# drprojects/DeepViewAgg

Measured on AMD Instinct MI355X. Metric: points/sec fused fwd+bwd (1M pts, 32 views), higher is better.
Workload: dtype bf16

## Files before the change

deepviewagg_amd/_lib.py:

```python
import ctypes
import os

_HERE = os.path.dirname(os.path.abspath(__file__))
LIB_PATH = os.environ.get("DVA_LIB_PATH") or os.path.join(_HERE, "csrc", "libdva_hip.so")

DVA_F32, DVA_BF16, DVA_F16 = 0, 1, 2
DVA_GRID_F32, DVA_GRID_F64, DVA_GRID_I32, DVA_GRID_I64 = 0, 1, 2, 3
DVA_SUM, DVA_MEAN, DVA_MAX, DVA_MIN = 0, 1, 2, 3
REDUCE_CODE = {"sum": DVA_SUM, "add": DVA_SUM, "mean": DVA_MEAN, "max": DVA_MAX, "min": DVA_MIN}
CAMERA_CODE = {
    "s3dis_equirectangular": 0,
    "scannet": 1,
    "kitti360_perspective": 2,
    "kitti360_fisheye": 3,
}

_ERRORS = {
    -1: "DVA_ERR_INVALID (bad argument)",
    -2: "DVA_ERR_UNSUPPORTED",
    -3: "DVA_ERR_LAUNCH (HIP runtime error)",
    -4: "DVA_ERR_OVERFLOW (composite key does not fit int64)",
}


# ... 83 lines not shown
    "dva_rowbn_apply": (ctypes.c_int, [_vp, _vp, _vp, _i64, _i32, _f32, _i32, _vp]),
    "dva_rowbn_bwd_stats": (ctypes.c_int, [_vp, _vp, _vp, _vp, _i64, _i32, _f32, _i32, _vp]),
    "dva_rowbn_bwd_apply": (ctypes.c_int, [_vp, _vp, _vp, _vp, _vp, _vp, _i64, _i32, _f32, _i32, _vp]),
    "dva_emod_rows_grid": (ctypes.c_int, [_i64, _i32, _i32]),
    "dva_emod_rows_fwd": (ctypes.c_int, [_vp] * 6 + [_i64, _i32, _i32, _f32, _i32, _vp]),
    "dva_emod_rows_bwd": (ctypes.c_int, [_vp] * 11 + [_i64, _i32, _i32, _f32, _f32, _i32, _vp]),
    "dva_emod_rows_dw_reduce": (ctypes.c_int, [_vp, _i32, _i32, _vp, _vp, _i32, _i32, _vp, _vp]),
    "dva_bn_finalize": (ctypes.c_int, [_vp, ctypes.c_double, _vp, _vp, _vp, _vp, _vp, _f32, _f32, _i32, _i32, _vp,
                                       _vp]),
    "dva_scale_f64": (ctypes.c_int, [_vp, ctypes.c_double, _vp, _i32, _vp]),
    "dva_chain_prep": (ctypes.c_int, [_vp, _vp, _vp, _i32, _vp, _vp, _i32, _vp, _vp]),
    "dva_chain_tile_count": (ctypes.c_int, [_vp, _vp, _i32, _vp, _vp]),
    "dva_chain_tile_build": (ctypes.c_int, [_vp, _vp, _i32, _vp, _vp, _vp]),
    "dva_chain_moments": (ctypes.c_int, [_vp, _i64, _vp, _i32, _vp, _vp, _vp]),
    "dva_chain_stats2": (ctypes.c_int, [_vp, _vp, _vp, _vp, _vp, _vp, _vp, _vp, _vp, _vp, _i64, _vp]),
    "dva_chain_pooled": (ctypes.c_int, [_vp, _vp, _vp, _vp, _i64, _vp]),
    "dva_chain_stats": (ctypes.c_int, [_i32, _vp, _vp, _vp, _vp, _vp, _vp, _vp, _vp, _vp, _vp, _i64, _i64, _vp]),
    "dva_chain_attn_fwd": (ctypes.c_int, [_vp] * 18 + [_i64, _i64, _i64, _i32, _i32, _i32, _f32, _vp]),
    "dva_chain_attn_bwd": (ctypes.c_int, [_vp] * 14 + [_i64, _i64, _i64, _i32, _i32, _i32, _f32, _vp]),
    "dva_chain_attn_fwd_dt": (ctypes.c_int, [_vp] * 18 + [_i64, _i64, _i64, _i32, _i32, _i32, _f32, _i32, _vp]),
    "dva_chain_attn_bwd_dt": (ctypes.c_int, [_vp] * 14 + [_i64, _i64, _i64, _i32, _i32, _i32, _f32, _i32, _vp]),
    "dva_chain_attn_bwd_f32": (ctypes.c_int, [_vp] * 14 + [_i64, _i64, _i64, _i32, _i32, _i32, _f32, _vp]),
    "dva_gather_segment_max_fwd": (ctypes.c_int, [_vp] * 5 + [_i64, _i64, _i64, _i32, _i32, _vp]),
    "dva_gather_segment_max_bwd": (ctypes.c_int, [_vp] * 8 + [_i64, _i64, _i64, _i32, _i32, _vp]),
    "dva_chain_keys_compat": (ctypes.c_int, [_vp] * 14 + [_i32, _f32, _i64, _i64, _vp]),
    "dva_chain_attn_fwd_keys": (ctypes.c_int, [_vp] * 12 + [_f32] + [_vp] * 8 + [_i64, _i64, _i64, _i32, _i32, _i32, _f32, _vp]),
    "dva_qkv_dquery": (ctypes.c_int, [_vp, _i32, _vp, _vp, _vp, _i64, _i64, _i32, _f32, _vp]),
    "dva_chain_score_stats_keys": (ctypes.c_int, [_vp] * 15 + [_i32, _f32, _i64, _i64, _vp]),
    "dva_chain_bwd_layer6_keys": (ctypes.c_int, [_vp] * 16 + [_i32, _f32, _i64, _i64, _vp]),
    "dva_qkv_compat": (ctypes.c_int, [_vp] * 4 + [_i64, _i32, _f32, _vp]),
    "dva_qkv_compat_bwd": (ctypes.c_int, [_vp] * 7 + [_i64, _i64, _i32, _f32, _vp]),
    "dva_plan_split_table_bytes": (ctypes.c_int64, [_i64, _i64]),
    "dva_plan_split_build": (ctypes.c_int, [_vp, _i64, _i64, _vp, _vp, _vp, _i64, _vp, _i64, _vp]),
    "dva_plan_split_sort_records": (ctypes.c_int, [_vp, _vp, _i64, _i64, _vp, _vp, _i64, _vp, _vp, _vp]),
    "dva_plan_split_sort_records32": (ctypes.c_int, [_vp, _vp, _i64, _i64, _vp, _i64, _vp, _vp]),
    "dva_plan_split_rows_grad": (ctypes.c_int, [_vp, _vp, _i64, _i64, _vp, _i64, _vp, _i32, _i32, _i32, _i32, _vp]),
    "dva_chain_score_stats": (ctypes.c_int, [_vp] * 14 + [_i32, _i64, _i64, _vp]),
    "dva_chain_bwd_layer": (ctypes.c_int, [_i32] + [_vp] * 22 + [_i32, _i64, _i64, _vp]),
    "dva_gather_bilinear_taps_anchor": (ctypes.c_int, [_vp, _vp, _i64, _i32, _i32, _i32, _vp, _vp, _vp, _vp]),
    "dva_bilinear_taps_cat": (ctypes.c_int, [_i32, _vp, _vp, _vp, _vp, _vp, _vp, _vp, _i64, _vp, _vp, _vp, _vp]),
    "dva_anchor_rows_sum": (ctypes.c_int, [_vp, _vp, _vp, _vp, _vp, _i64, _i64, _i32, _i32, _vp]),
    "dva_anchor_combine": (ctypes.c_int, [_vp, _vp, _i32, _i32, _i32, _i32, _vp]),
    "dva_anchor_fixup": (ctypes.c_int, [_vp, _vp, _vp, _vp, _vp, _i64, _i32, _i32, _i32, _i32, _i32, _vp]),
    "dva_anchor_rows_sum_bn": (ctypes.c_int, [_vp] * 10 + [_i64, _i64, _i32, _vp]),
    "dva_anchor_fixup_bn": (ctypes.c_int, [_vp] * 8 + [_i64, _i32, _i32, _i32, _i32, _vp]),
    "dva_emod_prep": (ctypes.c_int, [_vp, _i32, _vp, _vp]),
    "dva_emod_stats": (ctypes.c_int, [_i32] + [_vp] * 9 + [_i64, _i64, _i32, _vp]),
    "dva_emod_attn_fwd": (ctypes.c_int, [_vp] * 23 + [_i64, _i64, _i64, _i32, _i32, _i32, _f32, _vp]),
    "dva_emod_attn_bwd": (ctypes.c_int, [_vp] * 20 + [_i64, _i64, _i64, _i32, _i32, _i32, _f32, _vp]),
    "dva_emod_stats1_plan": (ctypes.c_int, [_vp] * 6 + [_i64, _i64, _i32, _vp]),
    "dva_emod_bwd": (ctypes.c_int, [_i32] + [_vp] * 16 + [_i64, _i64, _i64, _i32, _i32, _vp]),
    "dva_chain_route_stats": (ctypes.c_int, [_vp, _vp, _vp, _vp, _vp, _vp, _i64, _vp]),
    "dva_copy_ceiling": (ctypes.c_int, [_vp, _vp, _i64, _vp]),
    "dva_zero_unseen_rows": (ctypes.c_int, [_vp, _vp, _i64, _i64, _vp]),
    "dva_chain_bn_consts": (ctypes.c_int, [_vp, ctypes.c_double, _vp, _vp, _vp, _vp, _vp, ctypes.c_float, ctypes.c_float,
                                           _i32, _vp, _i32, _i32, _vp, _vp, _vp]),
    "dva_concat_cast_fwd": (ctypes.c_int, [_vp, _vp, _vp, _i64, _i32, _i32, _i32, _vp]),
    "dva_concat_cast_bwd": (ctypes.c_int, [_vp, _vp, _vp, _i64, _i32, _i32, _i32, _vp]),
    "dva_mapping_row_index": (ctypes.c_int, [_vp, _vp, _vp, _i32, ctypes.c_double, _i64, _i64, _i32, _i32, _i32, _vp, _vp]),
    "dva_view_gather_rows_grad_rec16_to": (ctypes.c_int, [_vp, _vp, _vp, _vp, _vp, _i32, _i64, _i64, _i32, _i32, _i32, _vp]),
    "dva_chain_tile_chunks": (ctypes.c_int, [_vp, _i64, _i64, _i32, _vp, _vp]),
    "dva_chain_tile_offsets": (ctypes.c_int, [_vp, _i32, _vp, _vp, _vp]),
    "dva_bn_bwd_consts": (ctypes.c_int, [_vp, _vp, ctypes.c_double, _i32, _vp, _vp, _vp, _i32, _vp]),
    "dva_chain3_prep": (ctypes.c_int, [_vp, _vp, _vp, _i32, _vp, _vp, _i32, _vp, _vp]),
    "dva_chain3_stats2": (ctypes.c_int, [_vp] * 11 + [_i64, _vp]),
    "dva_chain3_stats": (ctypes.c_int, [_i32] + [_vp] * 9 + [_i64, _i64, _vp]),
# ... 185 lines not shown
```

deepviewagg_amd/csrc/deepset.hip:

```cpp
#include "dva_common.h"

namespace dva {

constexpr int D = 32;
constexpr int TILE = 32;
constexpr float SLOPE = 0.2f;

struct BNc {
  float mean, invstd, gamma, beta;
};
__device__ __forceinline__ BNc load_bn(const float* __restrict__ bn, int c) {
  BNc b;
  b.mean = bn[c]; b.invstd = bn[D + c]; b.gamma = bn[2 * D + c]; b.beta = bn[3 * D + c];
  return b;
}
__device__ __forceinline__ float bn_hat(float a, const BNc& b) { return (a - b.mean) * b.invstd; }
__device__ __forceinline__ float bn_z(float a, const BNc& b) { return bn_hat(a, b) * b.gamma + b.beta; }
__device__ __forceinline__ float leaky(float z) { return z > 0.f ? z : SLOPE * z; }
__device__ __forceinline__ float dleaky(float z) { return z > 0.f ? 1.f : SLOPE; }

__device__ __forceinline__ void wave_sync() {
  asm volatile("s_waitcnt lgkmcnt(0)" ::: "memory");
  __builtin_amdgcn_wave_barrier();
}
// ... 543 lines not shown
      const int e = i * 64 + lane;
      const int64_t g = row0 * 8 + e;
      s_x[wv][e] = g < V * 8 ? x_map[g] : 0.f;
    }
    wave_sync();
#pragma unroll 4
    for (int i = 0; i < 16; ++i) {
      const int row = 2 * i + h;
      const int64_t r = row0 + row;
      if (r < V) {
        const float a1 = dot_row<8>(&s_x[wv][row * 8], wa);
        const float da = gsc * (Elt<AT>::ld(dz1, r * D + n) - s1m - bn_hat(a1, b) * s2m);
        const float4 x0 = *reinterpret_cast<const float4*>(&s_x[wv][row * 8]);
        const float4 x1 = *reinterpret_cast<const float4*>(&s_x[wv][row * 8 + 4]);
        acc[0] = fmaf(da, x0.x, acc[0]); acc[1] = fmaf(da, x0.y, acc[1]);
        acc[2] = fmaf(da, x0.z, acc[2]); acc[3] = fmaf(da, x0.w, acc[3]);
        acc[4] = fmaf(da, x1.x, acc[4]); acc[5] = fmaf(da, x1.y, acc[5]);
        acc[6] = fmaf(da, x1.z, acc[6]); acc[7] = fmaf(da, x1.w, acc[7]);
      }
    }
    wave_sync();
  }
  for (int i = threadIdx.x; i < D * 8; i += blockDim.x) s_red[i] = 0.f;
  __syncthreads();
#pragma unroll
  for (int k = 0; k < 8; ++k) {
    const float v = acc[k] + __shfl_xor(acc[k], 32);
    if (lane < 32) atomicAdd(&s_red[n * 8 + k], v);
  }
  __syncthreads();
  for (int i = threadIdx.x; i < D * 8; i += blockDim.x) atomicAdd(&dWa[i], s_red[i]);
}

__global__ __launch_bounds__(256) void csr_expand_kernel(const int64_t* __restrict__ ptr, int64_t N,
                                                          int32_t* __restrict__ vp) {
  const int lane = threadIdx.x & 63;
  const int64_t wave = ((int64_t)blockIdx.x * blockDim.x + threadIdx.x) >> 6;
  const int64_t n_waves = ((int64_t)gridDim.x * blockDim.x) >> 6;
  for (int64_t p0 = wave * 64; p0 < N; p0 += n_waves * 64) {
    const int64_t pl = p0 + lane < N ? p0 + lane : N - 1;
    const int64_t b = ptr[pl], e = ptr[pl + 1];
    const int n_here = (int)(N - p0 < 64 ? N - p0 : 64);
    const int64_t first = __shfl(b, 0), last = __shfl(e, n_here - 1);
    if (last - first <= 8 * n_here) {
      if (lane < n_here)
        for (int64_t r = b; r < e; ++r) vp[r] = (int32_t)(p0 + lane);
    } else {
      for (int i = 0; i < n_here; ++i) {
        const int64_t bi = __shfl(b, i), ei = __shfl(e, i);
        for (int64_t r = bi + lane; r < ei; r += 64) vp[r] = (int32_t)(p0 + i);
      }
    }
  }
}

static inline int grid_rows(int64_t V) {
  return capped_grid((V + TILE - 1) / TILE, 4, 256 * 8);
}

int dsm_launch_fwd_first(const float*, const float*, const float*, const float*, void*, double*, int64_t,
                         int, int, hipStream_t);
int dsm_launch_fwd_layer(const void*, const float*, const float*, const float*, const int32_t*, void*,
                         double*, int64_t, int, hipStream_t);
int dsm_launch_fwd_score(const void*, const float*, const float*, const float*, float*, int64_t, int,
                         const float*, const float*, int, hipStream_t);
int dsm_launch_bwd_layer(const void*, const void*, const float*, const float*, const float*, const void*,
                         const float*, const float*, void*, float*, double*, float*, const int32_t*, float*,
                         const float*, int64_t, int, int, int, hipStream_t);
int dsm_launch_bwd_max(const void*, const void*, const float*, const int32_t*, const float*, const int32_t*,
                       void*, double*, int64_t, int, hipStream_t);
int dsm_launch_bwd_score(const float*, const void*, const float*, const float*, void*, float*, float*,
                         double*, int64_t, int, const float*, const float*, int, hipStream_t);

static inline int act_bf(int32_t act_dtype) {
  return act_dtype == DVA_F32 ? 0 : act_dtype == DVA_BF16 ? 1 : -1;
}

}

using namespace dva;

extern "C" {

int dva_csr_expand(const int64_t* ptr, int64_t n_groups, int32_t* group_of_row, void* stream) {
  if (n_groups < 0 || !ptr) return DVA_ERR_INVALID;
  if (n_groups == 0) return DVA_OK;
  if (!group_of_row) return DVA_ERR_INVALID;
  int64_t b = (n_groups + 255) / 256;
  if (b > 8192) b = 8192;
  hipLaunchKernelGGL(csr_expand_kernel, dim3((int)b), dim3(256), 0, (hipStream_t)stream, ptr, n_groups,
                     group_of_row);
  DVA_CHECK_LAUNCH();
  return DVA_OK;
}

int dva_deepset_fwd_first(const float* x_map, const float* Wa, const float* bn1, const float* Wb,
                          void* a2_, double* stats, int64_t V, int32_t F, int32_t stats_only,
                          int32_t algo, int32_t act_dtype, void* stream) {
  const int bf = act_bf(act_dtype);
  if (act_dtype == DVA_F16) return DVA_ERR_UNSUPPORTED;
  if (V < 0 || !stats || bf < 0) return DVA_ERR_INVALID;
  if (bf && algo == 1) return DVA_ERR_UNSUPPORTED;
  float* a2 = (float*)a2_;
  if (F != 8) return DVA_ERR_UNSUPPORTED;
  if (V == 0) return DVA_OK;
  if (!x_map || !Wa) return DVA_ERR_INVALID;
  if (!stats_only && (!bn1 || !Wb || !a2)) return DVA_ERR_INVALID;
  hipStream_t s = (hipStream_t)stream;
  if (algo != 1) {
    dsm_launch_fwd_first(x_map, Wa, bn1, Wb, a2_, stats, V, stats_only, bf, s);
    DVA_CHECK_LAUNCH();
    return DVA_OK;
  }
  if (stats_only) {
    hipLaunchKernelGGL((dsf_fwd_first_kernel<true>), dim3(grid_rows(V)), dim3(256), 0, s, x_map, Wa,
                       (const float*)nullptr, (const float*)nullptr, (float*)nullptr, stats, V);
  } else {
    if (!bn1 || !Wb || !a2) return DVA_ERR_INVALID;
    hipLaunchKernelGGL((dsf_fwd_first_kernel<false>), dim3(grid_rows(V)), dim3(256), 0, s, x_map, Wa,
                       bn1, Wb, a2, stats, V);
  }
  DVA_CHECK_LAUNCH();
  return DVA_OK;
}
// ... 202 lines not shown
```

deepviewagg_amd/csrc/dva_common.h:

```cpp
#pragma once
#include <hip/hip_runtime.h>
#include <stdint.h>

#include "../../include/dva.h"

#define DVA_WAVE 64

#define DVA_CHECK_LAUNCH()                           \
  do {                                               \
    hipError_t e__ = hipGetLastError();              \
    if (e__ != hipSuccess) return DVA_ERR_LAUNCH;    \
  } while (0)

namespace dva {

typedef uint16_t bf16_t;

__device__ __forceinline__ float bf2f(bf16_t h) { return __uint_as_float(((uint32_t)h) << 16); }

typedef __bf16 dva_bf16x2 __attribute__((ext_vector_type(2)));
typedef float dva_f32x2 __attribute__((ext_vector_type(2)));
__device__ __forceinline__ uint32_t pack_bf16x2(float lo, float hi) {
  const dva_f32x2 v = {lo, hi};
  const dva_bf16x2 b = __builtin_convertvector(v, dva_bf16x2);
// ... 50 lines not shown
};
template <>
struct Elt<bf16_t> {
  static __device__ __forceinline__ float ld(const bf16_t* p, int64_t i) { return bf2f(p[i]); }
  static __device__ __forceinline__ void st(bf16_t* p, int64_t i, float v) { p[i] = f2bf(v); }
};
template <>
struct Elt<f16_t> {
  static __device__ __forceinline__ float ld(const f16_t* p, int64_t i) { return (float)p[i]; }
  static __device__ __forceinline__ void st(f16_t* p, int64_t i, float v) { p[i] = (f16_t)v; }
};

__host__ __device__ __forceinline__ int group_of_channel(int c, int C, int G) {
  if (G <= 1) return 0;
  if (G >= C) return c;
  const int base = C / G, rem = C % G;
  const int split = rem * (base + 1);
  return c < split ? c / (base + 1) : rem + (c - split) / base;
}
__host__ __device__ __forceinline__ int group_begin(int g, int C, int G) {
  if (g >= G) return C;
  if (G <= 1) return 0;
  if (G >= C) return g;
  const int base = C / G, rem = C % G;
  return g < rem ? g * (base + 1) : rem * (base + 1) + (g - rem) * base;
}

struct __attribute__((aligned(8))) PackedIdx {
  int32_t img;
  int16_t x;
  int16_t y;
};

static inline int blocks_for(int64_t n, int threads) { return (int)((n + threads - 1) / threads); }

static inline int capped_grid(int64_t n, int64_t per_block, int64_t cap) {
  int64_t b = (n + per_block - 1) / per_block;
  if (b > cap) b = cap;
  if (b < 1) b = 1;
  return (int)b;
}

static inline size_t align_up(size_t bytes, size_t align = 256) { return (bytes + align - 1) & ~(align - 1); }

class Carver {
 public:
  explicit Carver(void* base, size_t align = 256) : base_((uintptr_t)base), align_(align) {}
  template <typename T>
  T* take(size_t count) {
    T* p = (T*)(base_ + off_);
    off_ += align_up(count * sizeof(T), align_);
    return p;
  }
  size_t used() const { return off_; }

 private:
  uintptr_t base_;
  size_t off_ = 0, align_;
};

}
```

deepviewagg_amd/csrc/gather.hip:

```cpp
#include "dva_common.h"

namespace dva {

__device__ __forceinline__ float floordiv_f32(float a, float b) {
  const float mod = fmodf(a, b);
  float div = __fdiv_rn(__fsub_rn(a, mod), b);
  if (mod != 0.f && ((b < 0.f) != (mod < 0.f))) div = __fsub_rn(div, 1.f);
  if (div != 0.f) {
    float fl = floorf(div);
    if (__fsub_rn(div, fl) > 0.5f) fl = __fadd_rn(fl, 1.f);
    return fl;
  }
  return copysignf(0.f, __fdiv_rn(a, b));
}

template <typename PIX>
__global__ __launch_bounds__(256) void pack_index_kernel(const int64_t* __restrict__ images,
                                                          const int64_t* __restrict__ atom_ptr,
                                                          const PIX* __restrict__ pixels,
                                                          double ratio, int64_t n_views,
                                                          PackedIdx* __restrict__ out) {
  for (int64_t v = blockIdx.x * (int64_t)blockDim.x + threadIdx.x; v < n_views;
       v += (int64_t)gridDim.x * blockDim.x) {
    const int32_t img = (int32_t)images[v];
    for (int64_t a = atom_ptr[v]; a < atom_ptr[v + 1]; ++a) {
      PackedIdx pi;
      pi.img = img;
      if (ratio == 1.0) {
        pi.x = (int16_t)pixels[2 * a];
        pi.y = (int16_t)pixels[2 * a + 1];
      } else {
        const float rf = (float)ratio;
        pi.x = (int16_t)floordiv_f32((float)pixels[2 * a], rf);
        pi.y = (int16_t)floordiv_f32((float)pixels[2 * a + 1], rf);
      }
      out[a] = pi;
    }
  }
}

template <typename PIX>
__global__ __launch_bounds__(256) void mapping_row_index_kernel(const int64_t* __restrict__ images,
                                                                 const int64_t* __restrict__ atom_ptr,
                                                                 const PIX* __restrict__ pixels, double ratio,
                                                                 int64_t n_views, int H, int W,
                                                                 int32_t* __restrict__ row_idx) {
  for (int64_t v = blockIdx.x * (int64_t)blockDim.x + threadIdx.x; v < n_views;
// ... 839 lines not shown
```

deepviewagg_amd/csrc/plan_split.hip:

```cpp
#include "dva_common.h"

namespace dva {
namespace ps {

constexpr int IPT = 8;
constexpr int BINS = 512;
constexpr int LO_BITS = 9;
constexpr int HEAD_INTS = 4096;

constexpr int PLAN_TILE = 4096;

struct Layout {
  int64_t nt, nb, ntb;
  size_t off_tot, off_bstart, off_tstart, off_order, off_a, off_b, off_desc, total;
};

static inline bool eligible(int64_t n_views, int64_t n_rows) {
  return n_views > 0 && n_views <= 0x7fffffffLL && n_rows > BINS && n_rows <= (int64_t)BINS * BINS;
}

static inline Layout layout(int64_t n, int64_t n_rows) {
  Layout L;
  L.nt = (n + PLAN_TILE - 1) / PLAN_TILE;
  L.nb = (n_rows + BINS - 1) / BINS;
// ... 24 lines not shown
  int before = 0, all = 0;
#pragma unroll
  for (int i = 0; i < NT / 64; ++i) {
    const int t = s_w[i];
    before += i < w ? t : 0;
    all += t;
  }
  if (total) *total = all;
  return before + inc - v;
}

__device__ __forceinline__ int rfl_i(int v) { return __builtin_amdgcn_readfirstlane(v); }

__device__ __forceinline__ int hi_digit(uint32_t key, int nb) {
  const int d = (int)(key >> LO_BITS);
  return d < nb ? d : nb - 1;
}

template <int TILE>
__global__ __launch_bounds__(TILE / IPT) void hist_hi_kernel(const uint32_t* __restrict__ keys, int64_t n, int nb,
                                                             int64_t nt, int32_t* __restrict__ offA) {
  constexpr int THREADS = TILE / IPT;
  __shared__ int h[BINS];
  for (int i = threadIdx.x; i < BINS; i += THREADS) h[i] = 0;
  __syncthreads();
  const int64_t base = (int64_t)blockIdx.x * TILE;
#pragma unroll
  for (int k = 0; k < IPT; ++k) {
    const int64_t e = base + k * THREADS + threadIdx.x;
    if (e < n) atomicAdd(&h[hi_digit(keys[e], nb)], 1);
  }
  __syncthreads();
  for (int i = threadIdx.x; i < nb; i += THREADS) offA[(int64_t)i * nt + blockIdx.x] = h[i];
}

__global__ __launch_bounds__(256) void scan_tiles_kernel(int32_t* __restrict__ off, int64_t nt, int32_t* __restrict__ tot) {
  __shared__ int s_w[4];
  int32_t* row = off + (int64_t)blockIdx.x * nt;
  int carry = 0;
  for (int64_t t0 = 0; t0 < nt; t0 += 256) {
    const int64_t t = t0 + threadIdx.x;
    const int v = t < nt ? row[t] : 0;
    int all;
    const int ex = block_excl_scan<256>(v, s_w, &all);
    if (t < nt) row[t] = carry + ex;
    carry += all;
  }
  if (threadIdx.x == 0) tot[blockIdx.x] = carry;
}

__global__ __launch_bounds__(BINS) void bucket_starts_kernel(const int32_t* __restrict__ tot, int nb, int TILE,
                                                             int32_t* __restrict__ bucket_start,
                                                             int32_t* __restrict__ tile_start, int4* __restrict__ desc,
                                                             int32_t* __restrict__ order) {
  __shared__ int s_w[BINS / 64];
  __shared__ int s_tot[BINS];
  const int d = threadIdx.x;
  const int v = d < nb ? tot[d] : 0;
  s_tot[d] = d < nb ? v : -1;
  __syncthreads();
  if (d < nb) {
    int before = 0;
    for (int j = 0; j < nb; ++j) {
      const int t = s_tot[j];
      before += (t > v || (t == v && j < d)) ? 1 : 0;
    }
// ... 420 lines not shown
    }
  }
#pragma unroll
  for (int rr = 0; rr < RPT; ++rr) {
    const int64_t r = (int64_t)b * BINS + grp + GROUPS * rr;
    if (r < n_rows)
      *reinterpret_cast<float4*>(grows + r * C + cl * 4) = make_float4(acc[rr][0], acc[rr][1], acc[rr][2], acc[rr][3]);
  }
}

template <int C, typename T>
static void bucket_rows_grad(const uint4* rec, const T* gout, T* grows, int64_t n_rows, int G, int nb,
                             const int32_t* bstart, const int32_t* order, hipStream_t s) {
  hipLaunchKernelGGL((bucket_rows_grad_kernel<C, 8192, T>), dim3(nb), dim3(1024), 0, s, rec, gout, grows, n_rows, G, bstart, order);
}

}
}

namespace dva {
namespace ps {
struct Tables {
  int32_t *tot, *bstart, *tstart, *order, *offA, *offB;
  int4* desc;
};
static inline Tables tables_of(void* tables, const Layout& L) {
  char* tb = (char*)tables;
  return {(int32_t*)(tb + L.off_tot), (int32_t*)(tb + L.off_bstart), (int32_t*)(tb + L.off_tstart),
          (int32_t*)(tb + L.off_order), (int32_t*)(tb + L.off_a), (int32_t*)(tb + L.off_b), (int4*)(tb + L.off_desc)};
}

static inline unsigned scatter_grid(int64_t tiles) { return (unsigned)((tiles + 7) / 8 * 8); }

static void build(const uint32_t* keys, int64_t n, int64_t n_rows, int32_t* row_ptr, int32_t* counts, const Layout& L,
                  const Tables& T, void* scratch, hipStream_t s) {
  constexpr int TILE = PLAN_TILE, THREADS = TILE / IPT;
  const int nb = (int)L.nb;
  hipLaunchKernelGGL(hist_hi_kernel<TILE>, dim3((unsigned)L.nt), dim3(THREADS), 0, s, keys, n, nb, L.nt, T.offA);
  hipLaunchKernelGGL(scan_tiles_kernel, dim3(nb), dim3(256), 0, s, T.offA, L.nt, T.tot);
  hipLaunchKernelGGL(bucket_starts_kernel, dim3(1), dim3(BINS), 0, s, T.tot, nb, TILE, T.bstart, T.tstart, T.desc, T.order);
  hipLaunchKernelGGL((scatter_kernel<MODE_LOWS, TILE>), dim3(scatter_grid(L.nt)), dim3(THREADS), 0, s, keys,
                     (const uint4*)nullptr, scratch, n, nb, n_rows, L.nt, T.bstart, T.tstart, T.desc, T.offA,
                     (const int32_t*)nullptr);
  hipLaunchKernelGGL(hist_lo_kernel<TILE>, dim3((unsigned)L.ntb), dim3(THREADS), 0, s, (const uint16_t*)scratch, nb,
                     T.tstart, T.desc, T.offB);
  hipLaunchKernelGGL(scan_rows_kernel, dim3(nb), dim3(BINS), 0, s, T.offB, T.bstart, T.tstart, n_rows, n, row_ptr, counts);
}

static void sort_records(const uint32_t* keys, const uint4* rec, int64_t n, int64_t n_rows, const int32_t* row_ptr,
                         const Layout& L, const Tables& T, void* buf, void* out, hipStream_t s) {
  constexpr int TILE = PLAN_TILE, THREADS = TILE / IPT;
  const int nb = (int)L.nb;
  hipLaunchKernelGGL((scatter_kernel<MODE_REC_A, TILE>), dim3(scatter_grid(L.nt)), dim3(THREADS), 0, s, keys, rec,
                     buf, n, nb, n_rows, L.nt, T.bstart, T.tstart, T.desc, T.offA, (const int32_t*)nullptr);
  if (!out) return;
  hipLaunchKernelGGL((scatter_kernel<MODE_REC_B, TILE>), dim3(scatter_grid(L.ntb)), dim3(THREADS), 0, s,
                     (const uint32_t*)nullptr, (const uint4*)buf, out, n, nb, n_rows, L.nt, T.bstart, T.tstart, T.desc,
                     T.offB, row_ptr);
}
}
}

using namespace dva;

extern "C" {

int64_t dva_plan_split_table_bytes(int64_t n_views, int64_t n_rows) {
  if (n_views < 0 || n_rows < 0) return DVA_ERR_INVALID;
  if (!ps::eligible(n_views, n_rows)) return DVA_ERR_UNSUPPORTED;
  return (int64_t)ps::layout(n_views, n_rows).total;
}

int dva_plan_split_build(const int32_t* row_idx, int64_t n_views, int64_t n_rows, int32_t* row_ptr, int32_t* counts,
                         void* tables, int64_t tables_bytes, void* scratch, int64_t scratch_bytes, void* stream) {
  if (n_views < 0 || n_rows < 0) return DVA_ERR_INVALID;
  if (!ps::eligible(n_views, n_rows)) return DVA_ERR_UNSUPPORTED;
  if (!row_idx || !row_ptr || !tables || !scratch) return DVA_ERR_INVALID;
  const ps::Layout L = ps::layout(n_views, n_rows);
  if ((int64_t)L.total > tables_bytes || scratch_bytes < n_views * 2) return DVA_ERR_INVALID;
  const ps::Tables T = ps::tables_of(tables, L);
  ps::build((const uint32_t*)row_idx, n_views, n_rows, row_ptr, counts, L, T, scratch, (hipStream_t)stream);
  DVA_CHECK_LAUNCH();
  return DVA_OK;
}

int dva_plan_split_sort_records(const int32_t* row_idx, const void* rec, int64_t n_views, int64_t n_rows,
                                const int32_t* row_ptr, const void* tables, int64_t tables_bytes, void* buf,
                                void* rec_sorted, void* stream) {
  if (n_views < 0 || n_rows < 0) return DVA_ERR_INVALID;
  if (!ps::eligible(n_views, n_rows)) return DVA_ERR_UNSUPPORTED;
  if (!rec || !row_ptr || !tables || !buf || buf == rec || buf == rec_sorted) return DVA_ERR_INVALID;
  if (((uintptr_t)rec % 16) || ((uintptr_t)buf % 16) || ((uintptr_t)rec_sorted % 16)) return DVA_ERR_UNSUPPORTED;
  const ps::Layout L = ps::layout(n_views, n_rows);
  if ((int64_t)L.total > tables_bytes) return DVA_ERR_INVALID;
  const ps::Tables T = ps::tables_of(const_cast<void*>(tables), L);
  ps::sort_records((const uint32_t*)row_idx, (const uint4*)rec, n_views, n_rows, row_ptr, L, T, buf, rec_sorted,
                   (hipStream_t)stream);
  DVA_CHECK_LAUNCH();
  return DVA_OK;
}

int dva_plan_split_sort_records32(const int32_t* row_idx, const void* rec, int64_t n_views, int64_t n_rows,
                                  const void* tables, int64_t tables_bytes, void* buf, void* stream) {
  if (n_views < 0 || n_rows < 0) return DVA_ERR_INVALID;
  if (!ps::eligible(n_views, n_rows)) return DVA_ERR_UNSUPPORTED;
  if (!row_idx || !rec || !tables || !buf || buf == rec) return DVA_ERR_INVALID;
  if (((uintptr_t)rec % 16) || ((uintptr_t)buf % 16)) return DVA_ERR_UNSUPPORTED;
  const ps::Layout L = ps::layout(n_views, n_rows);
  if ((int64_t)L.total > tables_bytes) return DVA_ERR_INVALID;
  const ps::Tables T = ps::tables_of(const_cast<void*>(tables), L);
  constexpr int TILE = ps::PLAN_TILE, THREADS = TILE / ps::IPT;
  hipLaunchKernelGGL((ps::scatter_kernel<ps::MODE_REC_A, TILE, 8>), dim3(ps::scatter_grid(L.nt)), dim3(THREADS), 0,
                     (hipStream_t)stream, (const uint32_t*)row_idx, (const uint4*)rec, buf, n_views, (int)L.nb, n_rows,
                     L.nt, T.bstart, T.tstart, T.desc, T.offA, (const int32_t*)nullptr);
// ... 48 lines not shown
```

deepviewagg_amd/csrc/segment.hip:

```cpp
#include "dva_common.h"

namespace dva {

template <typename T, int REDUCE>
__global__ __launch_bounds__(256) void segment_csr_fwd_kernel(const T* __restrict__ src,
                                                               const int64_t* __restrict__ ptr,
                                                               T* __restrict__ out,
                                                               int32_t* __restrict__ arg,
                                                               int64_t n_groups, int C) {
  const int64_t total = n_groups * (int64_t)C;
  for (int64_t t = blockIdx.x * (int64_t)blockDim.x + threadIdx.x; t < total;
       t += (int64_t)gridDim.x * blockDim.x) {
    const int64_t g = t / C;
    const int c = (int)(t - g * C);
    const int64_t beg = ptr[g], end = ptr[g + 1];
    float acc;
    int64_t best = -1;
    if (REDUCE == DVA_SUM || REDUCE == DVA_MEAN) {
      acc = 0.f;
      for (int64_t r = beg; r < end; ++r) acc += Elt<T>::ld(src, r * C + c);
      if (REDUCE == DVA_MEAN && end > beg) acc /= (float)(end - beg);
    } else {
      acc = 0.f;
      for (int64_t r = beg; r < end; ++r) {
// ... 257 lines not shown
}

template <typename T>
static int launch_segment_bwd(const void* gout, const int64_t* ptr, const int32_t* arg, void* gsrc,
                              int64_t n, int C, int reduce, hipStream_t s) {
  const bool vec = vec_ok<T>(gout, gsrc, C);
  const int grid = capped_grid(n * (int64_t)(vec ? C / SVec<T>::N : C), 256, CSR_GRID_CAP);
#define DVA_L(R)                                                                                         \
  do {                                                                                                   \
    if (vec)                                                                                             \
      hipLaunchKernelGGL((segment_csr_bwd_vec_kernel<T, R>), dim3(grid), dim3(256), 0, s, (const T*)gout, \
                         ptr, arg, (T*)gsrc, n, C);                                                      \
    else                                                                                                 \
      hipLaunchKernelGGL((segment_csr_bwd_kernel<T, R>), dim3(grid), dim3(256), 0, s, (const T*)gout,    \
                         ptr, arg, (T*)gsrc, n, C);                                                      \
  } while (0)
  switch (reduce) {
    case DVA_SUM: DVA_L(DVA_SUM); break;
    case DVA_MEAN: DVA_L(DVA_MEAN); break;
    case DVA_MAX: DVA_L(DVA_MAX); break;
    case DVA_MIN: DVA_L(DVA_MIN); break;
    default: return DVA_ERR_INVALID;
  }
#undef DVA_L
  return DVA_OK;
}

}

using namespace dva;

extern "C" {

int dva_version(void) { return 321; }

int dva_device_count(void) {
  int n = 0;
  hipError_t e = hipGetDeviceCount(&n);
  if (e == hipErrorNoDevice) return 0;
  if (e != hipSuccess) return DVA_ERR_LAUNCH;
  return n;
}

int dva_segment_csr_fwd(const void* src, const int64_t* ptr, void* out, int32_t* arg,
                        int64_t n_groups, int32_t C, int32_t dtype, int32_t reduce, void* stream) {
  if (n_groups < 0 || C < 0 || !ptr) return DVA_ERR_INVALID;
  if (reduce < DVA_SUM || reduce > DVA_MIN) return DVA_ERR_INVALID;
  if (n_groups == 0 || C == 0) return DVA_OK;
  if (!out) return DVA_ERR_INVALID;
  int rc;
  if (dtype == DVA_F32)
    rc = launch_segment_fwd<float>(src, ptr, out, arg, n_groups, C, reduce, (hipStream_t)stream);
  else if (dtype == DVA_BF16)
    rc = launch_segment_fwd<bf16_t>(src, ptr, out, arg, n_groups, C, reduce, (hipStream_t)stream);
  else if (dtype == DVA_F16)
    rc = launch_segment_fwd<f16_t>(src, ptr, out, arg, n_groups, C, reduce, (hipStream_t)stream);
  else
    return DVA_ERR_INVALID;
  if (rc) return rc;
  DVA_CHECK_LAUNCH();
  return DVA_OK;
}

int dva_segment_csr_bwd(const void* grad_out, const int64_t* ptr, const int32_t* arg,
                        void* grad_src, int64_t n_groups, int32_t C, int32_t dtype,
                        int32_t reduce, void* stream) {
  if (n_groups < 0 || C < 0 || !ptr) return DVA_ERR_INVALID;
// ... 71 lines not shown
```

deepviewagg_amd/ops.py:

```python
import collections
import os

import threading

import numpy as np
import torch

from . import _lib
from ._lib import check, dtype_code, ptr, require_device, stream_of

ROWS_GRAD_ALGO = 0
ATTENTION_ALGO = 0


class KernelTimer:

    def __init__(self, only=None):
        self.records = []
        self.only = None if only is None else set(only)

    def launch(self, name, nbytes):
        if self.only is not None and name not in self.only:
            return _NO_TIMER
        return _TimedLaunch(self, name, nbytes)
# ... 640 lines not shown
    with _timed("view_gather_rows_grad", V * ((4 if perm is not None else 0) + 16 + C * 2) + R * (C * 2 + 4)):
        check(lib.dva_view_gather_rows_grad_rec16_to(ptr(gout), ptr(perm), ptr(row_ptr), ptr(rec), ptr(g), dtype_code(g),
                                                     R, V, C, G, dtype_code(gout), stream),
              "dva_view_gather_rows_grad_rec16_to")
    return g


def csr_expand(csr_idx, n_views):
    lib = _lib.load()
    require_device(csr_idx)
    vp = torch.empty(n_views, dtype=torch.int32, device=csr_idx.device)
    check(lib.dva_csr_expand(ptr(csr_idx), csr_idx.shape[0] - 1, ptr(vp), stream_of(csr_idx)),
          "dva_csr_expand")
    return vp


def gather_row_index(packed_idx, B, H, W, row_offset=0, with_counts=True, with_plan=False, split=True):
    lib = _lib.load()
    require_device(packed_idx)
    P = packed_idx.shape[0]
    row_idx = torch.empty(P, dtype=torch.int32, device=packed_idx.device)
    hist = with_counts and not with_plan
    counts = torch.zeros(B * H * W, dtype=torch.int32, device=packed_idx.device) if hist else None
    with _timed("gather_row_index", P * 12):
        check(lib.dva_gather_row_index(ptr(packed_idx), P, B, H, W, int(row_offset), ptr(row_idx),
                                       ptr(counts), stream_of(packed_idx)), "dva_gather_row_index")
    if with_plan:
        assert row_offset == 0, "a plan is built over the rows of one map"
        plan, counts = row_plan(row_idx, B * H * W, with_counts, split)
        return row_idx, counts, plan
    return row_idx, counts


def mapping_row_index(images, atom_ptr, pixels, ratio, B, H, W, with_counts=True, with_plan=True, split=True):
    lib = _lib.load()
    require_device(images, atom_ptr, pixels)
    images = images.contiguous()
    atom_ptr = _check_ptr(atom_ptr)
    pixels = pixels.contiguous()
    if pixels.dtype not in (torch.int16, torch.int32, torch.int64):
        raise TypeError(f"pixels must be int16/int32/int64, got {pixels.dtype}")
    V, P = images.shape[0], pixels.shape[0]
    row_idx = torch.empty(P, dtype=torch.int32, device=pixels.device)
    with _timed("gather_row_index", V * 28 + P * 8):
        check(lib.dva_mapping_row_index(ptr(images), ptr(atom_ptr), ptr(pixels), pixels.element_size(), float(ratio),
                                        V, P, B, H, W, ptr(row_idx), stream_of(pixels)), "dva_mapping_row_index")
    if not with_plan:
        return row_idx, None, None
    plan, counts = row_plan(row_idx, B * H * W, with_counts, split)
    return row_idx, counts, plan


class GatheredFeatures:

    def __init__(self, rows, row_idx, counts, exact, plan=None):
        self.rows, self.row_idx, self.counts, self.exact = rows, row_idx, counts, exact
        self.plan = plan

    def with_rows(self, rows):
        assert rows.shape[0] == self.rows.shape[0]
        plan = self.plan
        if isinstance(plan, SplitPlan) and not split_plan_serves(rows.dtype, rows.shape[1]):
            plan = None
        return GatheredFeatures(rows, self.row_idx, self.counts, self.exact, plan)

    @property
    def shape(self):
        return torch.Size((self.row_idx.shape[0], self.rows.shape[1]))

    @property
    def device(self):
        return self.rows.device

    @property
# ... 7 lines not shown
        return gather_rows(self.rows, self.row_idx)

    @staticmethod
    def cat(items, order=None):
        offs, rows, idx, cnt = 0, [], [], []
        for it in items:
            rows.append(it.rows)
            idx.append(it.row_idx + offs)
            cnt.append(it.counts)
            offs += it.rows.shape[0]
        if len(items) == 1 and order is None:
            return items[0]
        row_idx = torch.cat(idx)
        if order is not None:
            row_idx = row_idx[order]
        return GatheredFeatures(torch.cat(rows, dim=0), row_idx.contiguous(), torch.cat(cnt),
                                all(it.exact for it in items))


def lazy_gather_nearest(x, packed_idx, exact):
    assert x.dim() == 4
    B, C, H, W = x.shape
    rows = x.permute(0, 2, 3, 1).reshape(B * H * W, C)
    row_idx, counts, plan = gather_row_index(packed_idx, B, H, W, with_plan=True,
                                             split=bool(exact) and split_plan_serves(x.dtype, C))
    return GatheredFeatures(rows, row_idx, counts, exact, plan)


def lazy_gather_nearest_mapping(x, images, atom_ptr, pixels, ratio, exact):
    assert x.dim() == 4
    B, C, H, W = x.shape
    rows = x.permute(0, 2, 3, 1).reshape(B * H * W, C)
    row_idx, counts, plan = mapping_row_index(images, atom_ptr, pixels, ratio, B, H, W,
                                              split=bool(exact) and split_plan_serves(x.dtype, C))
    return GatheredFeatures(rows, row_idx, counts, exact, plan)


class _GatherSegmentMax(torch.autograd.Function):

    @staticmethod
    def forward(ctx, rows, row_idx, atom_ptr, plan):
        lib = _lib.load()
        require_device(rows, row_idx, atom_ptr)
        rows = rows.contiguous()
        (R, C), V, P = rows.shape, atom_ptr.shape[0] - 1, row_idx.shape[0]
        out = torch.empty((V, C), dtype=rows.dtype, device=rows.device)
        arg = torch.empty((V, C), dtype=torch.int16, device=rows.device)
        es = rows.element_size()
        with _timed("gather_segment_max_fwd", P * (4 + C * es) + V * (8 + C * (es + 2))):
            check(lib.dva_gather_segment_max_fwd(ptr(rows), ptr(row_idx), ptr(atom_ptr), ptr(out), ptr(arg), V, P, R, C,
                                                 dtype_code(rows), stream_of(rows)), "dva_gather_segment_max_fwd")
        ctx.save_for_backward(row_idx, atom_ptr, arg)
        ctx.meta = (R, C, rows.dtype)
        ctx.plan = plan
        return out

    @staticmethod
    def backward(ctx, gout):
        lib = _lib.load()
        row_idx, atom_ptr, arg = ctx.saved_tensors
        R, C, dt = ctx.meta
        gout = gout.contiguous().to(dt)
        V, P = atom_ptr.shape[0] - 1, row_idx.shape[0]
        es = gout.element_size()
        groups = C // (16 // es)
        if SEGMENT_MAX_ATOMICS or groups & (groups - 1) or groups > 64 or P > 0x7fffffff:
            grows = torch.zeros((R, C), dtype=torch.float32, device=gout.device)
# ... 1738 lines not shown
```

include/dva.h:

```cpp
#ifndef DVA_H_
#define DVA_H_

#include <stdint.h>

#ifdef __cplusplus
extern "C" {
#endif

#define DVA_OK 0
#define DVA_ERR_INVALID (-1)
#define DVA_ERR_UNSUPPORTED (-2)
#define DVA_ERR_LAUNCH (-3)
#define DVA_ERR_OVERFLOW (-4)

#define DVA_F32 0
#define DVA_BF16 1
#define DVA_F16 2

#define DVA_SUM 0
#define DVA_MEAN 1
#define DVA_MAX 2
#define DVA_MIN 3

#define DVA_CAM_EQUIRECT 0
// ... 59 lines not shown

int dva_view_attention_bwd(const void* grad_out, const void* val, const float* compat,
                           const float* att, const float* gate, const int32_t* amax,
                           const int64_t* ptr, const float* gate_w, const float* gate_b,
                           void* grad_val, float* grad_compat, float* grad_gate_wb,
                           int64_t n_points, int64_t n_views, int32_t C, int32_t G, int32_t scaling,
                           int32_t dtype, int32_t algo, void* stream);

int dva_view_gather_attention_fwd(const void* rows, const int32_t* row_idx, const float* compat,
                                  const int64_t* ptr, const float* gate_w, const float* gate_b,
                                  void* out, float* att, float* gate, int32_t* amax,
                                  int64_t n_points, int64_t n_views, int32_t C, int32_t G,
                                  int32_t scaling, float eps, int32_t dtype, int32_t algo,
                                  void* stream);
int dva_view_gather_attention_bwd(const void* grad_out, const void* rows, const int32_t* row_idx,
                                  const float* compat, const float* att, const float* gate,
                                  const int32_t* amax, const int64_t* ptr, const float* gate_w,
                                  const float* gate_b, float* grad_rows, float* grad_compat,
                                  float* grad_gate_wb, float* view_rec, int32_t rec_stride,
                                  int64_t n_points, int64_t n_views, int32_t C, int32_t G,
                                  int32_t scaling, int32_t dtype, int32_t algo, void* stream);

int dva_view_attention_geometry(int32_t C, int32_t G, int64_t n_points, int64_t n_views, int32_t dtype, int32_t* lpr,
                                int32_t* rows);

int64_t dva_row_plan_workspace_bytes(int64_t n_views, int64_t n_rows);
int dva_row_plan(const int32_t* row_idx, int64_t n_views, int64_t n_rows, int32_t* perm,
                 int32_t* row_ptr, int32_t* counts, void* workspace, int64_t workspace_bytes,
                 void* stream);

int64_t dva_plan_split_table_bytes(int64_t n_views, int64_t n_rows);
int dva_plan_split_build(const int32_t* row_idx, int64_t n_views, int64_t n_rows, int32_t* row_ptr, int32_t* counts,
                         void* tables, int64_t tables_bytes, void* scratch, int64_t scratch_bytes, void* stream);
int dva_plan_split_sort_records(const int32_t* row_idx, const void* rec, int64_t n_views, int64_t n_rows,
                                const int32_t* row_ptr, const void* tables, int64_t tables_bytes, void* buf,
                                void* rec_sorted, void* stream);
int dva_plan_split_sort_records32(const int32_t* row_idx, const void* rec, int64_t n_views, int64_t n_rows,
                                  const void* tables, int64_t tables_bytes, void* buf, void* stream);
int dva_plan_split_rows_grad(const void* grad_out, const void* bucket_rec, int64_t n_views, int64_t n_rows,
                             const void* tables, int64_t tables_bytes, void* grad_rows, int32_t C, int32_t G, int32_t dtype,
                             int32_t out_dtype, void* stream);

int dva_view_gather_rows_grad(const void* grad_out, const float* att, const float* gate,
                              const int32_t* view_point, const int32_t* perm, const int32_t* row_ptr,
                              const float* view_rec, int32_t rec_stride, float* grad_rows,
                              int64_t n_rows, int64_t n_views, int32_t C, int32_t G, int32_t dtype,
                              void* stream);

int dva_view_gather_rows_grad_rec16_to(const void* grad_out, const int32_t* perm, const int32_t* row_ptr,
                                       const void* view_rec16, void* grad_rows, int32_t out_dtype, int64_t n_rows,
                                       int64_t n_views, int32_t C, int32_t G, int32_t dtype, void* stream);

int dva_gather_rows_sum(const void* grad_out, const int32_t* perm, const int32_t* row_ptr,
                        const float* weights, int32_t atom_shift, float* grad_rows, int64_t n_rows,
                        int64_t n_atoms, int32_t C, int32_t dtype, void* stream);
int dva_gather_bilinear_taps_anchor(const void* packed_idx, const float* coords, int64_t n_atoms, int32_t B,
                                    int32_t H, int32_t W, int32_t* rows, float* weights, int32_t* anchors,
                                    void* stream);
int dva_bilinear_taps_cat(int32_t n_settings, const void* const* tap_rows, const void* const* tap_weights,
                          const void* const* anchors, const int64_t* n_views, const int64_t* n_rows,
                          const int64_t* n_anchors, const int64_t* order, int64_t n_views_total, int32_t* rows_out,
                          float* weights_out, int32_t* anchors_out, void* stream);
int dva_anchor_rows_sum(const void* grad_out, const int32_t* perm, const int32_t* row_ptr, const float* weights,
                        float* S, int64_t n_anchors, int64_t n_views, int32_t C, int32_t dtype, void* stream);
int dva_anchor_combine(const float* S, float* grad_rows, int32_t B, int32_t H, int32_t W, int32_t C, void* stream);
int dva_anchor_fixup(const void* grad, const int32_t* rows, const float* weights, const int32_t* anchors,
// ... 424 lines not shown
```

Before: 105.0 million.

## Fuse mapping row-index computation with split-plan histogram; vectorize CSR expand

Adds a fused kernel that computes pixel row keys from image/pixel mappings and builds the high-digit per-tile histogram in the same pass. This removes the separate row-index kernel and the re-read of keys by hist_hi, and optionally processes several tiles per block. Separately, the CSR expand kernel's dense branch now writes aligned int4 chunks using a wave-wide binary search instead of per-group strided scalar stores. The fused path is used only when exact mode and the split plan apply, and it adds alignment and eligibility checks that fall back to the old path otherwise.

```diff
diff --git a/deepviewagg_amd/_lib.py b/deepviewagg_amd/_lib.py
--- a/deepviewagg_amd/_lib.py
+++ b/deepviewagg_amd/_lib.py
@@ -139,6 +139,8 @@
     "dva_qkv_compat_bwd": (ctypes.c_int, [_vp] * 7 + [_i64, _i64, _i32, _f32, _vp]),
     "dva_plan_split_table_bytes": (ctypes.c_int64, [_i64, _i64]),
     "dva_plan_split_build": (ctypes.c_int, [_vp, _i64, _i64, _vp, _vp, _vp, _i64, _vp, _i64, _vp]),
+    "dva_mapping_row_index_split": (ctypes.c_int, [_vp, _vp, _i32, ctypes.c_double, _i64, _i32, _i32, _i32, _vp, _vp, _vp, _vp,
+                                                   _i64, _vp, _i64, _vp]),
     "dva_plan_split_sort_records": (ctypes.c_int, [_vp, _vp, _i64, _i64, _vp, _vp, _i64, _vp, _vp, _vp]),
     "dva_plan_split_sort_records32": (ctypes.c_int, [_vp, _vp, _i64, _i64, _vp, _i64, _vp, _vp]),
     "dva_plan_split_rows_grad": (ctypes.c_int, [_vp, _vp, _i64, _i64, _vp, _i64, _vp, _i32, _i32, _i32, _i32, _vp]),
diff --git a/deepviewagg_amd/csrc/deepset.hip b/deepviewagg_amd/csrc/deepset.hip
--- a/deepviewagg_amd/csrc/deepset.hip
+++ b/deepviewagg_amd/csrc/deepset.hip
@@ -599,8 +599,15 @@
   for (int i = threadIdx.x; i < D * 8; i += blockDim.x) atomicAdd(&dWa[i], s_red[i]);
 }
 
+__device__ __forceinline__ int last_start_at_most(int start, int o) {
+  int pos = 0;
+#pragma unroll
+  for (int step = 32; step; step >>= 1) pos += __shfl(start, pos + step) <= o ? step : 0;
+  return pos;
+}
+
 __global__ __launch_bounds__(256) void csr_expand_kernel(const int64_t* __restrict__ ptr, int64_t N,
-                                                          int32_t* __restrict__ vp) {
+                                                          int32_t* __restrict__ vp, int vp_mis) {
   const int lane = threadIdx.x & 63;
   const int64_t wave = ((int64_t)blockIdx.x * blockDim.x + threadIdx.x) >> 6;
   const int64_t n_waves = ((int64_t)gridDim.x * blockDim.x) >> 6;
@@ -613,9 +620,27 @@
       if (lane < n_here)
         for (int64_t r = b; r < e; ++r) vp[r] = (int32_t)(p0 + lane);
     } else {
-      for (int i = 0; i < n_here; ++i) {
-        const int64_t bi = __shfl(b, i), ei = __shfl(e, i);
-        for (int64_t r = bi + lane; r < ei; r += 64) vp[r] = (int32_t)(p0 + i);
+      for (int64_t r0 = first - ((first + vp_mis) & 3); r0 < last; r0 += 256) {
+        const int64_t rb = b - r0;
+        const int start = lane < n_here ? (int)(rb < 0 ? 0 : rb > 256 ? 256 : rb) : 256;
+        const int o = lane * 4;
+        int pt[4];
+        pt[0] = last_start_at_most(start, o);
+        pt[3] = last_start_at_most(start, o + 3);
+        pt[1] = pt[2] = pt[0];
+        if (__any(pt[0] != pt[3])) {
+          pt[1] = last_start_at_most(start, o + 1);
+          pt[2] = last_start_at_most(start, o + 2);
+        }
+        const int64_t r = r0 + o;
+        const int32_t base = (int32_t)p0;
+        if (r >= first && r + 4 <= last) {
+          *reinterpret_cast<int4*>(vp + r) = make_int4(base + pt[0], base + pt[1], base + pt[2], base + pt[3]);
+        } else {
+#pragma unroll
+          for (int j = 0; j < 4; ++j)
+            if (r + j >= first && r + j < last) vp[r + j] = base + pt[j];
+        }
       }
     }
   }
@@ -656,7 +681,7 @@
   int64_t b = (n_groups + 255) / 256;
   if (b > 8192) b = 8192;
   hipLaunchKernelGGL(csr_expand_kernel, dim3((int)b), dim3(256), 0, (hipStream_t)stream, ptr, n_groups,
-                     group_of_row);
+                     group_of_row, (int)(((uintptr_t)group_of_row >> 2) & 3));
   DVA_CHECK_LAUNCH();
   return DVA_OK;
 }
diff --git a/deepviewagg_amd/csrc/dva_common.h b/deepviewagg_amd/csrc/dva_common.h
--- a/deepviewagg_amd/csrc/dva_common.h
+++ b/deepviewagg_amd/csrc/dva_common.h
@@ -106,6 +106,18 @@
   int16_t y;
 };
 
+__device__ __forceinline__ float floordiv_f32(float a, float b) {
+  const float mod = fmodf(a, b);
+  float div = __fdiv_rn(__fsub_rn(a, mod), b);
+  if (mod != 0.f && ((b < 0.f) != (mod < 0.f))) div = __fsub_rn(div, 1.f);
+  if (div != 0.f) {
+    float fl = floorf(div);
+    if (__fsub_rn(div, fl) > 0.5f) fl = __fadd_rn(fl, 1.f);
+    return fl;
+  }
+  return copysignf(0.f, __fdiv_rn(a, b));
+}
+
 static inline int blocks_for(int64_t n, int threads) { return (int)((n + threads - 1) / threads); }
 
 static inline int capped_grid(int64_t n, int64_t per_block, int64_t cap) {
diff --git a/deepviewagg_amd/csrc/gather.hip b/deepviewagg_amd/csrc/gather.hip
--- a/deepviewagg_amd/csrc/gather.hip
+++ b/deepviewagg_amd/csrc/gather.hip
@@ -1,18 +1,6 @@
 #include "dva_common.h"
 
 namespace dva {
-
-__device__ __forceinline__ float floordiv_f32(float a, float b) {
-  const float mod = fmodf(a, b);
-  float div = __fdiv_rn(__fsub_rn(a, mod), b);
-  if (mod != 0.f && ((b < 0.f) != (mod < 0.f))) div = __fsub_rn(div, 1.f);
-  if (div != 0.f) {
-    float fl = floorf(div);
-    if (__fsub_rn(div, fl) > 0.5f) fl = __fadd_rn(fl, 1.f);
-    return fl;
-  }
-  return copysignf(0.f, __fdiv_rn(a, b));
-}
 
 template <typename PIX>
 __global__ __launch_bounds__(256) void pack_index_kernel(const int64_t* __restrict__ images,
diff --git a/deepviewagg_amd/csrc/plan_split.hip b/deepviewagg_amd/csrc/plan_split.hip
--- a/deepviewagg_amd/csrc/plan_split.hip
+++ b/deepviewagg_amd/csrc/plan_split.hip
@@ -80,6 +80,65 @@
   }
   __syncthreads();
   for (int i = threadIdx.x; i < nb; i += THREADS) offA[(int64_t)i * nt + blockIdx.x] = h[i];
+}
+
+#ifndef DVA_PLAN_FUSED_K
+#define DVA_PLAN_FUSED_K 16
+#endif
+constexpr int FUSED_K = DVA_PLAN_FUSED_K;
+
+template <typename PIX>
+struct __attribute__((aligned(2 * sizeof(PIX)))) PixPair {
+  PIX x, y;
+};
+
+template <typename PIX, int TILE, int K>
+__global__ __launch_bounds__(TILE / IPT) void mapping_row_index_kernel_hist(const int64_t* __restrict__ images,
+                                                                            const PixPair<PIX>* __restrict__ pixels,
+                                                                            double ratio, int64_t n, int H, int W, int nb,
+                                                                            int64_t nt, int32_t* __restrict__ row_idx,
+                                                                            int32_t* __restrict__ offA) {
+  constexpr int THREADS = TILE / IPT, HS = BINS + 1;
+  __shared__ int h[K * HS];
+  for (int i = threadIdx.x; i < K * HS; i += THREADS) h[i] = 0;
+  __syncthreads();
+  const int64_t t0 = (int64_t)blockIdx.x * K;
+  const float rf = (float)ratio;
+  for (int j = 0; j < K && t0 + j < nt; ++j) {
+    const int64_t base = (t0 + j) * TILE;
+    int64_t im[IPT];
+    PixPair<PIX> px[IPT];
+#pragma unroll
+    for (int k = 0; k < IPT; ++k) {
+      const int64_t e = base + k * THREADS + threadIdx.x;
+      const int64_t g = e < n ? e : n - 1;
+      im[k] = images[g];
+      px[k] = pixels[g];
+    }
+#pragma unroll
+    for (int k = 0; k < IPT; ++k) {
+      const int64_t e = base + k * THREADS + threadIdx.x;
+      const int32_t img = (int32_t)im[k];
+      int32_t x, y;
+      if (ratio == 1.0) {
+        x = (int32_t)px[k].x;
+        y = (int32_t)px[k].y;
+      } else {
+        x = (int32_t)(int16_t)floordiv_f32((float)px[k].x, rf);
+        y = (int32_t)(int16_t)floordiv_f32((float)px[k].y, rf);
+      }
+      const int32_t key = (img * H + y) * W + x;
+      if (e < n) {
+        row_idx[e] = key;
+        atomicAdd(&h[j * HS + hi_digit((uint32_t)key, nb)], 1);
+      }
+    }
+  }
+  __syncthreads();
+  for (int i = threadIdx.x; i < nb * K; i += THREADS) {
+    const int d = i / K, j = i % K;
+    if (t0 + j < nt) offA[(int64_t)d * nt + t0 + j] = h[j * HS + d];
+  }
 }
 
 __global__ __launch_bounds__(256) void scan_tiles_kernel(int32_t* __restrict__ off, int64_t nt, int32_t* __restrict__ tot) {
@@ -566,11 +625,10 @@
 
 static inline unsigned scatter_grid(int64_t tiles) { return (unsigned)((tiles + 7) / 8 * 8); }
 
-static void build(const uint32_t* keys, int64_t n, int64_t n_rows, int32_t* row_ptr, int32_t* counts, const Layout& L,
-                  const Tables& T, void* scratch, hipStream_t s) {
+static void build_tail(const uint32_t* keys, int64_t n, int64_t n_rows, int32_t* row_ptr, int32_t* counts, const Layout& L,
+                       const Tables& T, void* scratch, hipStream_t s) {
   constexpr int TILE = PLAN_TILE, THREADS = TILE / IPT;
   const int nb = (int)L.nb;
-  hipLaunchKernelGGL(hist_hi_kernel<TILE>, dim3((unsigned)L.nt), dim3(THREADS), 0, s, keys, n, nb, L.nt, T.offA);
   hipLaunchKernelGGL(scan_tiles_kernel, dim3(nb), dim3(256), 0, s, T.offA, L.nt, T.tot);
   hipLaunchKernelGGL(bucket_starts_kernel, dim3(1), dim3(BINS), 0, s, T.tot, nb, TILE, T.bstart, T.tstart, T.desc, T.order);
   hipLaunchKernelGGL((scatter_kernel<MODE_LOWS, TILE>), dim3(scatter_grid(L.nt)), dim3(THREADS), 0, s, keys,
@@ -579,6 +637,28 @@
   hipLaunchKernelGGL(hist_lo_kernel<TILE>, dim3((unsigned)L.ntb), dim3(THREADS), 0, s, (const uint16_t*)scratch, nb,
                      T.tstart, T.desc, T.offB);
   hipLaunchKernelGGL(scan_rows_kernel, dim3(nb), dim3(BINS), 0, s, T.offB, T.bstart, T.tstart, n_rows, n, row_ptr, counts);
+}
+
+static void build(const uint32_t* keys, int64_t n, int64_t n_rows, int32_t* row_ptr, int32_t* counts, const Layout& L,
+                  const Tables& T, void* scratch, hipStream_t s) {
+  constexpr int TILE = PLAN_TILE;
+  hipLaunchKernelGGL(hist_hi_kernel<TILE>, dim3((unsigned)L.nt), dim3(TILE / IPT), 0, s, keys, n, (int)L.nb, L.nt, T.offA);
+  build_tail(keys, n, n_rows, row_ptr, counts, L, T, scratch, s);
+}
+
+template <typename PIX>
+static void build_from_mapping(const int64_t* images, const void* pixels, double ratio, int64_t n, int H, int W,
+                               int64_t n_rows, int32_t* row_idx, int32_t* row_ptr, int32_t* counts, const Layout& L,
+                               const Tables& T, void* scratch, hipStream_t s) {
+  constexpr int TILE = PLAN_TILE;
+  if (L.nt >= (int64_t)FUSED_K * 512)
+    hipLaunchKernelGGL((mapping_row_index_kernel_hist<PIX, TILE, FUSED_K>), dim3((unsigned)((L.nt + FUSED_K - 1) / FUSED_K)),
+                       dim3(TILE / IPT), 0, s, images, (const PixPair<PIX>*)pixels, ratio, n, H, W, (int)L.nb, L.nt,
+                       row_idx, T.offA);
+  else
+    hipLaunchKernelGGL((mapping_row_index_kernel_hist<PIX, TILE, 1>), dim3((unsigned)L.nt), dim3(TILE / IPT), 0, s, images,
+                       (const PixPair<PIX>*)pixels, ratio, n, H, W, (int)L.nb, L.nt, row_idx, T.offA);
+  build_tail((const uint32_t*)row_idx, n, n_rows, row_ptr, counts, L, T, scratch, s);
 }
 
 static void sort_records(const uint32_t* keys, const uint4* rec, int64_t n, int64_t n_rows, const int32_t* row_ptr,
@@ -614,6 +694,31 @@
   if ((int64_t)L.total > tables_bytes || scratch_bytes < n_views * 2) return DVA_ERR_INVALID;
   const ps::Tables T = ps::tables_of(tables, L);
   ps::build((const uint32_t*)row_idx, n_views, n_rows, row_ptr, counts, L, T, scratch, (hipStream_t)stream);
+  DVA_CHECK_LAUNCH();
+  return DVA_OK;
+}
+
+int dva_mapping_row_index_split(const int64_t* images, const void* pixels, int32_t pix_bytes, double ratio,
+                                int64_t n_views, int32_t B, int32_t H, int32_t W, int32_t* row_idx, int32_t* row_ptr,
+                                int32_t* counts, void* tables, int64_t tables_bytes, void* scratch, int64_t scratch_bytes,
+                                void* stream) {
+  if (n_views < 0 || !(ratio >= 1.0) || B < 0 || H < 0 || W < 0) return DVA_ERR_INVALID;
+  if (pix_bytes != 2 && pix_bytes != 4 && pix_bytes != 8) return DVA_ERR_INVALID;
+  if (H > 32767 || W > 32767) return DVA_ERR_UNSUPPORTED;
+  const int64_t n_rows = (int64_t)B * H * W;
+  if (!ps::eligible(n_views, n_rows)) return DVA_ERR_UNSUPPORTED;
+  if (!images || !pixels || !row_idx || !row_ptr || !tables || !scratch) return DVA_ERR_INVALID;
+  if ((uintptr_t)pixels % (2 * (size_t)pix_bytes)) return DVA_ERR_UNSUPPORTED;
+  const ps::Layout L = ps::layout(n_views, n_rows);
+  if ((int64_t)L.total > tables_bytes || scratch_bytes < n_views * 2) return DVA_ERR_INVALID;
+  const ps::Tables T = ps::tables_of(tables, L);
+  hipStream_t s = (hipStream_t)stream;
+  if (pix_bytes == 2)
+    ps::build_from_mapping<int16_t>(images, pixels, ratio, n_views, H, W, n_rows, row_idx, row_ptr, counts, L, T, scratch, s);
+  else if (pix_bytes == 4)
+    ps::build_from_mapping<int32_t>(images, pixels, ratio, n_views, H, W, n_rows, row_idx, row_ptr, counts, L, T, scratch, s);
+  else
+    ps::build_from_mapping<int64_t>(images, pixels, ratio, n_views, H, W, n_rows, row_idx, row_ptr, counts, L, T, scratch, s);
   DVA_CHECK_LAUNCH();
   return DVA_OK;
 }
diff --git a/deepviewagg_amd/csrc/segment.hip b/deepviewagg_amd/csrc/segment.hip
--- a/deepviewagg_amd/csrc/segment.hip
+++ b/deepviewagg_amd/csrc/segment.hip
@@ -313,7 +313,7 @@
 
 extern "C" {
 
-int dva_version(void) { return 321; }
+int dva_version(void) { return 322; }
 
 int dva_device_count(void) {
   int n = 0;
diff --git a/deepviewagg_amd/ops.py b/deepviewagg_amd/ops.py
--- a/deepviewagg_amd/ops.py
+++ b/deepviewagg_amd/ops.py
@@ -696,7 +696,28 @@
     return row_idx, counts
 
 
-def mapping_row_index(images, atom_ptr, pixels, ratio, B, H, W, with_counts=True, with_plan=True, split=True):
+def _mapping_row_index_split(images, pixels, ratio, B, H, W, with_counts):
+    lib = _lib.load()
+    V, R, dev = images.shape[0], B * H * W, pixels.device
+    es = pixels.element_size()
+    if not (SPLIT_PLAN and _split_plan_pays(V, R)) or pixels.shape[0] != V or pixels.data_ptr() % (2 * es):
+        return None
+    nbytes = int(lib.dva_plan_split_table_bytes(V, R))
+    if nbytes <= 0:
+        return None
+    row_idx = torch.empty(V, dtype=torch.int32, device=dev)
+    row_ptr = torch.empty(R + 1, dtype=torch.int32, device=dev)
+    counts = torch.empty(R, dtype=torch.int32, device=dev) if with_counts else None
+    tables = torch.empty(nbytes, dtype=torch.uint8, device=dev)
+    lows = torch.empty(V, dtype=torch.int16, device=dev)
+    with _timed("mapping_row_plan", V * (8 + 2 * es + 4 + 4 + 4)):
+        check(lib.dva_mapping_row_index_split(ptr(images), ptr(pixels), es, float(ratio), V, B, H, W, ptr(row_idx),
+                                              ptr(row_ptr), ptr(counts), ptr(tables), nbytes, ptr(lows), V * 2,
+                                              stream_of(pixels)), "dva_mapping_row_index_split")
+    return row_idx, counts, SplitPlan(row_idx, R, row_ptr, tables)
+
+
+def mapping_row_index(images, atom_ptr, pixels, ratio, B, H, W, with_counts=True, with_plan=True, split=True, exact=False):
     lib = _lib.load()
     require_device(images, atom_ptr, pixels)
     images = images.contiguous()
@@ -704,6 +725,10 @@
     pixels = pixels.contiguous()
     if pixels.dtype not in (torch.int16, torch.int32, torch.int64):
         raise TypeError(f"pixels must be int16/int32/int64, got {pixels.dtype}")
+    if exact and split and with_plan:
+        fused = _mapping_row_index_split(images, pixels, ratio, B, H, W, with_counts)
+        if fused is not None:
+            return fused
     V, P = images.shape[0], pixels.shape[0]
     row_idx = torch.empty(P, dtype=torch.int32, device=pixels.device)
     with _timed("gather_row_index", V * 28 + P * 8):
@@ -777,7 +802,7 @@
     B, C, H, W = x.shape
     rows = x.permute(0, 2, 3, 1).reshape(B * H * W, C)
     row_idx, counts, plan = mapping_row_index(images, atom_ptr, pixels, ratio, B, H, W,
-                                              split=bool(exact) and split_plan_serves(x.dtype, C))
+                                              split=bool(exact) and split_plan_serves(x.dtype, C), exact=bool(exact))
     return GatheredFeatures(rows, row_idx, counts, exact, plan)
 
 
diff --git a/include/dva.h b/include/dva.h
--- a/include/dva.h
+++ b/include/dva.h
@@ -115,6 +115,10 @@
 int64_t dva_plan_split_table_bytes(int64_t n_views, int64_t n_rows);
 int dva_plan_split_build(const int32_t* row_idx, int64_t n_views, int64_t n_rows, int32_t* row_ptr, int32_t* counts,
                          void* tables, int64_t tables_bytes, void* scratch, int64_t scratch_bytes, void* stream);
+int dva_mapping_row_index_split(const int64_t* images, const void* pixels, int32_t pix_bytes, double ratio,
+                                int64_t n_views, int32_t B, int32_t H, int32_t W, int32_t* row_idx, int32_t* row_ptr,
+                                int32_t* counts, void* tables, int64_t tables_bytes, void* scratch, int64_t scratch_bytes,
+                                void* stream);
 int dva_plan_split_sort_records(const int32_t* row_idx, const void* rec, int64_t n_views, int64_t n_rows,
                                 const int32_t* row_ptr, const void* tables, int64_t tables_bytes, void* buf,
                                 void* rec_sorted, void* stream);
```

Measured after the change: 106.5 million, median of 6. 1.01x the previous value.
